# marekrams/tnac4o

Hardware: AMD Instinct MI355X
Metric: PEPS-contraction ms/sweep, chimera L=2048 chi=64 (boundary-MPS sweep _setup_rhoT) (lower is better)
Workload: dtype f64; 1 GPU; chimera L=2048 (Nx=Ny=16, Nc=8), synthetic couplings seed 20260004, beta=3, chi=64; one sweep = 16 rows of MPO absorb + compress_mps; one step = the sweeps of the 4 lattice rotations of one instance; parallelism=1 GPU: 4 lattice rotations of one instance interleaved on 4 HIP streams, mode=sweep

## Files before the change

### tnac4o_amd/csrc/common.h

```cpp
#pragma once
#include <hip/hip_runtime.h>
#include <stdint.h>
#include <stdio.h>
#include <stdlib.h>
#include <string.h>

namespace tn {

void set_error(const char* fmt, ...);
const char* get_error();

inline int hip_fail(hipError_t e, const char* what) {
    set_error("%s: %s", what, hipGetErrorString(e));
    return (int)e > 0 ? (int)e : 1;
}

#define TN_CHECK_ARG(cond, msg)                \
    do {                                       \
        if (!(cond)) {                         \
            tn::set_error("%s: %s", __func__, msg); \
            return -1;                         \
        }                                      \
    } while (0)

#define TN_CHECK_LAUNCH(what)                          \
    do {                                               \
        hipError_t e__ = hipGetLastError();            \
        if (e__ != hipSuccess) return tn::hip_fail(e__, what); \
    } while (0)

inline const char* env_str(const char* name) { return getenv(name); }
inline bool env_flag_on(const char* name) { const char* e = getenv(name); return !(e && e[0] == '0'); }
inline bool env_flag_set(const char* name) { const char* e = getenv(name); return e && e[0] == '1'; }
inline int env_int(const char* name, int dflt) { const char* e = getenv(name); return e ? atoi(e) : dflt; }
inline int64_t env_i64(const char* name, int64_t dflt) { const char* e = getenv(name); return e ? (int64_t)atoll(e) : dflt; }
inline double env_double(const char* name, double dflt) { const char* e = getenv(name); return e ? atof(e) : dflt; }

enum PinSlot {
    PIN_QR = 0,
    PIN_SVD_READ = 2,
    PIN_SVD_UPLOAD = 3,
    PIN_CHAIN_PACK = 4,
    PIN_CHAIN_UPLOAD = 5,
    PIN_CHAIN_READ = 6,
    PIN_SHARED = 7,
    PIN_NSLOTS
};
void* pinned_host(size_t bytes, PinSlot slot);
int read_back(hipStream_t st, void* host, const void* dev, size_t bytes, PinSlot slot, const char* what);
int read_back_staged(hipStream_t st, void** data, const void* dev, size_t bytes, PinSlot slot, const char* what);
int upload(hipStream_t st, void* dev, const void* host, size_t bytes, PinSlot slot, const char* what);

static inline int64_t cdiv(int64_t a, int64_t b) { return (a + b - 1) / b; }
static inline int64_t align_up(int64_t a, int64_t b) { return cdiv(a, b) * b; }

struct WsCarve {
    char* base;
    int64_t off = 0;
    template <typename T = char>
    T* take(int64_t bytes) {
        char* p = base ? base + off : nullptr;
        off += align_up(bytes, 256);
        return (T*)p;
    }
    int64_t total() const { return off; }
};
constexpr int64_t NORMALIZE_SCRATCH_BYTES = 8192;

enum { PROF_GEMM_128x128 = 0, PROF_GEMM_128x32, PROF_GEMM_32x128, PROF_GEMM_64x64, PROF_SPLITK_REDUCE, PROF_ABSORB,
       PROF_GRAM, PROF_EIG, PROF_ROWS_SMALL, PROF_VECS_SMALL,
       PROF_PANEL,
       PROF_LU,
       PROF_QR_AUX,
       PROF_SVD_AUX,
       PROF_MISC,
       PROF_NKERNEL,
       PROF_QR_NOMINAL = PROF_NKERNEL,
       PROF_SVD_NOMINAL,
       PROF_SVD_STREAM,
       PROF_SVDVALS_NOMINAL,
       PROF_SVD_ROUNDS,
       PROF_NFAM };
enum { PH_OTHER = 0, PH_ABSORB, PH_QR, PH_SVD, PH_SVDVALS, PH_BUILD, PH_N };
bool prof_on(int fam);
void prof_begin(hipStream_t st, int fam);
void prof_end(hipStream_t st, int fam, double flops, double bytes);
void prof_note(int fam, double calls, double flops, double bytes);
void prof_note_qr(int64_t m, int64_t n, int64_t batch);
void prof_note_svd(int64_t k, int64_t n, int sweeps);
void prof_note_svdvals(int64_t k, int64_t n);
int prof_phase(int phase);
struct ProfPhase {
    int prev;
    explicit ProfPhase(int ph) : prev(prof_phase(ph)) {}
    ~ProfPhase() { prof_phase(prev); }
};
#define TN_PROF_LAUNCH(st, fam, launch) do { prof_begin(st, fam); launch; prof_end(st, fam, 0.0, 0.0); } while (0)
void prof_set_mask(unsigned mask);
void prof_set_sample(unsigned n);
void prof_reset();
void prof_get(int phase, int fam, uint64_t* calls, double* ms, double* flops, double* bytes);

struct Mat {
    double* p;
    int64_t rs, cs;
};
static inline Mat mat(double* p, int64_t rs, int64_t cs) { return Mat{p, rs, cs}; }
static inline Mat sub(Mat a, int64_t i, int64_t j) { return Mat{a.p + i * a.rs + j * a.cs, a.rs, a.cs}; }
static inline Mat tr(Mat a) { return Mat{a.p, a.cs, a.rs}; }

int gemm(hipStream_t st, int64_t M, int64_t N, int64_t K, double alpha, const double* A, int64_t rsa, int64_t csa,
         const double* B, int64_t rsb, int64_t csb, double beta, double* C, int64_t rsc, int64_t csc,
         int64_t batch = 1, int64_t bsa = 0, int64_t bsb = 0, int64_t bsc = 0, double* ws = nullptr,
         int64_t ws_bytes = 0);
int64_t gemm_ws_bytes(int64_t M, int64_t N, int64_t K, int64_t batch);
struct GemmExtra {
    const int* pairs = nullptr;
    const int* skip = nullptr;
    int pw = 0, mapA = 0, mapB = 0, mapC = 0;
    int force_splitk = 0;
    bool raw_partials = false;
    int* splitk_used = nullptr;
};
int gemm_forced_split(int64_t K, int s, int64_t* kchunk);
int gemm_ex(hipStream_t st, int64_t M, int64_t N, int64_t K, double alpha, const double* A, int64_t rsa, int64_t csa,
            const double* B, int64_t rsb, int64_t csb, double beta, double* C, int64_t rsc, int64_t csc, int64_t batch,
            int64_t bsa, int64_t bsb, int64_t bsc, double* ws, int64_t ws_bytes, const GemmExtra* x);

static inline int gemm(hipStream_t st, int64_t M, int64_t N, int64_t K, double alpha, Mat A, Mat B, double beta, Mat C,
                       double* ws = nullptr, int64_t ws_bytes = 0) {
    return gemm(st, M, N, K, alpha, A.p, A.rs, A.cs, B.p, B.rs, B.cs, beta, C.p, C.rs, C.cs, 1, 0, 0, 0, ws, ws_bytes);
}
int gemm_prof_family(int64_t M, int64_t N, int64_t K, int64_t rsc, int64_t csc);

int rank_update(hipStream_t st, int64_t m, int64_t n, int b, const double* W, int64_t wrs, int64_t wcs, const double* X, int64_t xrs,
                int64_t xcs, double* C, int64_t rsc, int64_t csc, const int* active);
static inline int rank_update(hipStream_t st, int64_t m, int64_t n, int b, Mat W, Mat X, Mat C, const int* active = nullptr) {
    return rank_update(st, m, n, b, W.p, W.rs, W.cs, X.p, X.rs, X.cs, C.p, C.rs, C.cs, active);
}

struct FactorProducts {
    int64_t Z, I, J, K1, N, Mhi, Mlo;
    const double* P; int64_t pz, pi, pk;
    const double* X; int64_t xk, xj, xn;
    const double* W; int64_t wm, wq;
    double* Out; int64_t oz, ohi, olo, on;
};
bool factor_products_fits(int64_t Z, int64_t I, int64_t J, int64_t K1, int64_t N, int64_t M);
inline bool factor_products_on() { return env_flag_on("TN_FACTOR_FUSED"); }
int factor_products(hipStream_t st, const FactorProducts& f);

constexpr int NBMAX = 64;

int gram_partial(hipStream_t st, const double* X, int64_t vs, int64_t es, int64_t L, int nvec, int w, const int* pairs,
                 int ngroups, int nchunk, double* part);
int gram_nchunk(int64_t L);

int eig_small(hipStream_t st, const double* part, int nchunk, int nvec, int ngroups, int mode, int max_sweeps,
              double dead_thresh, double* out, int* dead, int* nrot, double* maxoff, double relevant2 = 0.0, int allow_fast = 1);

int rows_times_small(hipStream_t st, double* X, int64_t rs, int64_t cs, int64_t nrows, int b, const double* S);

struct SvdRoundsJob {
    double* X; int64_t pitch, L; int nvp, w;
    const int* pairs; int ng, nr, nchunk;
    double* part; int64_t part_bytes; double* Js; int* nrot; double* maxoff;
    double relevant2, last_tol; int inner_first, inner_later;
    double* norms;
};
int svd_rounds_fused(hipStream_t st, const SvdRoundsJob& j);
int small_t_times_vecs(hipStream_t st, const double* S, double* X, int64_t vs, int64_t es, int64_t L, int nvec, int w,
                       const int* pairs, int ngroups, const int* nrot);


int qr_factor(hipStream_t st, double* A, int64_t rs, int64_t cs, int64_t m, int64_t n, double* Q, int64_t qrs, int64_t qcs, double* R,
              int64_t rrs, int64_t rcs, int nb, void* ws, int64_t ws_bytes, double rank_tol, int64_t* keff_host,
              double* dropped2_host = nullptr, int frob_exit = 0, int64_t* pivot_perm_host = nullptr, double* nf_out2 = nullptr,
              int* nf_done = nullptr);
int64_t qr_ws_bytes(int64_t m, int64_t n, int nb);


constexpr int CQ_MAXPASS = 4;
constexpr double CQ_THETA = 1e-10;
constexpr double CQ_DONE = 5e-15;
constexpr double CQ_LAST = 1e-8;
int64_t cholqr_ws_bytes(int64_t nrows, int b);
int cholqr_reset(hipStream_t st, void* ws);
int cholqr_begin(hipStream_t st, void* ws, void** state_out);
void cholqr_end_ok(hipStream_t st);
int cholqr_orthonormalize(hipStream_t st, const double* X, int64_t irs, int64_t ics, double* Y, int64_t rs, int64_t cs, int64_t nrows,
                          int b, void* ws, int64_t ws_bytes, uint64_t seed, int* fused_base, void* state = nullptr);
int cholqr_panel(hipStream_t st, const double* X, int64_t irs, int64_t ics, double* Y, int64_t rs, int64_t cs, int64_t nrows, int b, void* ws,
                 int64_t ws_bytes, uint64_t seed, int reconstruct, double* Tp, double* W, int64_t wrs, int64_t wcs, double* Wq, int* fused_base,
                 void* state = nullptr, const int* active = nullptr);
int cholqr_debug_state(hipStream_t st, const void* ws, int* ints9, double* dev_hist);
int cholqr_stats(unsigned long long* out16, int reset, hipStream_t st_or_null, int all_streams);
bool smallqr_fits(int64_t m, int64_t n);
int64_t smallqr_ws_bytes(int64_t m, int64_t n);
int smallqr_factor(hipStream_t st, const double* A, int64_t rs, int64_t cs, int64_t m, int64_t n, double* Q, int64_t qrs, int64_t qcs, double* R,
                   int64_t rrs, int64_t rcs, double* nf_out2, void* ws, int64_t ws_bytes);

constexpr int CQ_FUSED_MAXBLK = 32;
constexpr unsigned CQ_SPIN_LIMIT = 1u << 22;
constexpr int CHOLQR_SLOTS = 64;
int cholqr_stream_slot(hipStream_t st);
void* device_pool_slot(const void* symbol, size_t slot_bytes, int slot);
unsigned panel_spin_limit();
int panel_maxpass();
int fused_maxblk();
bool fused_forms_allowed(hipStream_t st, int nwg);
void fused_forms_disable(hipStream_t st);
void fused_stream_released(hipStream_t st);
struct FusedTallLaunch {
    FusedTallLaunch(hipStream_t st, bool wanted);
    ~FusedTallLaunch();
    FusedTallLaunch(const FusedTallLaunch&) = delete;
// ... 98 lines not shown
```

### tnac4o_amd/csrc/devprim.h

```cpp
#pragma once
#include "common.h"

namespace tn {

static __device__ __forceinline__ double ld_agent(const double* p) { return __hip_atomic_load(p, __ATOMIC_RELAXED, __HIP_MEMORY_SCOPE_AGENT); }
static __device__ __forceinline__ int ldi_agent(const int* p) { return __hip_atomic_load(p, __ATOMIC_RELAXED, __HIP_MEMORY_SCOPE_AGENT); }
static __device__ __forceinline__ void st_agent(double* p, double v) { __hip_atomic_store(p, v, __ATOMIC_RELAXED, __HIP_MEMORY_SCOPE_AGENT); }
static __device__ __forceinline__ void sti_agent(int* p, int v) { __hip_atomic_store(p, v, __ATOMIC_RELAXED, __HIP_MEMORY_SCOPE_AGENT); }
static __device__ __forceinline__ void publish_wait() { __builtin_amdgcn_fence(__ATOMIC_RELEASE, "workgroup"); __builtin_amdgcn_s_waitcnt(0); }

template <int SLEEP>
static __device__ __forceinline__ bool grid_barrier(int* counter, int target, int* s_flag, int tid, unsigned spin_limit, int naps = 0) {
    publish_wait();
    __syncthreads();
    if (tid == 0) {
        atomicAdd(counter, 1);
        int ok = 1;
        unsigned spins = 0;
        while (ldi_agent(counter) < target) {
            __builtin_amdgcn_s_sleep(SLEEP);
            for (int i = 0; i < naps; ++i) __builtin_amdgcn_s_sleep(15);
            if (++spins > spin_limit) { ok = 0; break; }
        }
        *s_flag = ok;
    }
    __syncthreads();
    return *s_flag != 0;
}

static __device__ __forceinline__ double readlane_f64(double v, int lane) {
    int lo = __double2loint(v), hi = __double2hiint(v);
    lo = __builtin_amdgcn_readlane(lo, lane);
    hi = __builtin_amdgcn_readlane(hi, lane);
    return __hiloint2double(hi, lo);
}
static __device__ __forceinline__ double rsqrt2(double x) {
    double r = __builtin_amdgcn_rsq(x);
    r = r * (1.5 - 0.5 * x * r * r);
    r = r * (1.5 - 0.5 * x * r * r);
    return r;
}
static __device__ __forceinline__ double fast_rsqrt(double x) {
    double r = __builtin_amdgcn_rsq(x);
    r = r * (1.5 - 0.5 * x * r * r);
    r = r * (1.5 - 0.5 * x * r * r);
    r = r * (1.5 - 0.5 * x * r * r);
    return r;
}
static __device__ __forceinline__ double fast_rcp(double x) {
    double r = __builtin_amdgcn_rcp(x);
    r = r * (2.0 - x * r);
    r = r * (2.0 - x * r);
    r = r * (2.0 - x * r);
    return r;
}
static __device__ __forceinline__ void fnma(double& acc, double a, double b) {
    asm volatile("v_fma_f64 %0, -%1, %2, %0" : "+v"(acc) : "v"(a), "v"(b));
}
static __device__ __forceinline__ void fnma_s(double& acc, double s_uniform, double v) {
    asm volatile("v_fma_f64 %0, -%1, %2, %0" : "+v"(acc) : "s"(s_uniform), "v"(v));
}
static __device__ __forceinline__ double hash_unit(uint64_t x) {
    x ^= x >> 33; x *= 0xff51afd7ed558ccdULL; x ^= x >> 33; x *= 0xc4ceb9fe1a85ec53ULL; x ^= x >> 33;
    return ((double)(x >> 11) * (1.0 / 9007199254740992.0)) - 0.5;
}
static __device__ __forceinline__ void block_rows(int64_t nrows, int nblk, int blk, int64_t& r0, int& nr) {
    const int64_t base = nrows / nblk, rem = nrows % nblk;
    r0 = blk * base + (blk < rem ? blk : rem);
    nr = (int)(base + (blk < rem ? 1 : 0));
}

static __device__ __forceinline__ double block_sum(double v, double* red, int tid) {
#pragma unroll
    for (int o = 32; o > 0; o >>= 1) v += __shfl_xor(v, o, 64);
    __syncthreads();
    if ((tid & 63) == 0) red[tid >> 6] = v;
    __syncthreads();
    return (red[0] + red[1]) + (red[2] + red[3]);
}
static __device__ __forceinline__ double block_tree_sum(double v, double* red) {
    const int tid = threadIdx.x;
    red[tid] = v;
    __syncthreads();
    for (int k = 128; k > 0; k >>= 1) {
        if (tid < k) red[tid] += red[tid + k];
        __syncthreads();
    }
    const double r = red[0];
    __syncthreads();
    return r;
}
static __device__ __forceinline__ double block_tree_min(double v, double* red) {
    const int tid = threadIdx.x;
    red[tid] = v;
    __syncthreads();
    for (int k = 128; k > 0; k >>= 1) {
        if (tid < k) red[tid] = fmin(red[tid], red[tid + k]);
        __syncthreads();
    }
    const double r = red[0];
    __syncthreads();
    return r;
}

}
```

### tnac4o_amd/csrc/factor_products.hip

```cpp
#include "common.h"

namespace tn {

namespace {

typedef double d4 __attribute__((ext_vector_type(4)));

constexpr int FP_NC = 64;
constexpr int FP_QMAX = 256;
constexpr int FP_IMAX = 16;
constexpr int FP_K1MAX = 64;
constexpr int FP_THREADS = 512, FP_WAVES = FP_THREADS / 64;
constexpr int FP_SLAB = 32 * FP_WAVES;

struct FacP {
    const double* P;
    const double* X;
    const double* W;
    double* Out;
    int Z, I, J, K1, N, M, Mlo, chunks;
    int64_t pz, pi, pk, xk, xj, xn, wm, wq, oz, ohi, olo, on;
};

__device__ __forceinline__ int fp_sidx(int q, int c) { return q * FP_NC + (c ^ ((q & 1) << 4)); }

__device__ __forceinline__ double fp_keep(double v, bool keep) {
    long long m = keep ? -1ll : 0ll;
    asm volatile("" : "+v"(m));
    return __longlong_as_double(__double_as_longlong(v) & m);
}

template <int KS>
__device__ __forceinline__ void fp_stage1(const FacP& g, double* S, const int z, const int n0, const int nb, const int wave, const int lr, const int lk) {
    constexpr int KG = 4 * KS;
    double p[KG];
    {
        const double* Pz = g.P + (int64_t)z * g.pz + (int64_t)min(lr, g.I - 1) * g.pi;
#pragma unroll
        for (int kk = 0; kk < KG; ++kk) {
            const int k = kk * 4 + lk;
            const double v = Pz[(int64_t)min(k, g.K1 - 1) * g.pk];
            p[kk] = fp_keep(v, lr < g.I && k < g.K1);
        }
    }
    const int units = g.J * nb;
    auto load = [&](double (&b)[KG], const int u) {
        const int uc = min(u, units - 1), j = uc / nb, cb = uc - j * nb, n = n0 + cb * 16 + lr;
        const double* Xp = g.X + (int64_t)j * g.xj + (int64_t)min(n, g.N - 1) * g.xn;
#pragma unroll
        for (int kk = 0; kk < KG; ++kk) {
            const int k = kk * 4 + lk;
            const double v = Xp[(int64_t)min(k, g.K1 - 1) * g.xk];
            b[kk] = fp_keep(v, n < g.N && k < g.K1);
        }
    };
    auto multiply = [&](const double (&b)[KG], const int u) {
        if (u >= units) return;
        d4 acc = d4{0.0, 0.0, 0.0, 0.0};
#pragma unroll
        for (int kk = 0; kk < KG; ++kk) acc = __builtin_amdgcn_mfma_f64_16x16x4f64(p[kk], b[kk], acc, 0, 0, 0);
        const int j = u / nb, cb = u - j * nb;
#pragma unroll
        for (int r = 0; r < 4; ++r) {
            const int i = lk + 4 * r;
            if (i < g.I) S[fp_sidx(i * g.J + j, cb * 16 + lr)] = acc[r];
        }
    };
    double b0[KG], b1[KG];
    load(b0, wave);
    for (int u = wave; u < units; u += 2 * FP_WAVES) {
        load(b1, u + FP_WAVES);
        multiply(b0, u);
        load(b0, u + 2 * FP_WAVES);
        multiply(b1, u + FP_WAVES);
    }
}

template <int TN>
__device__ __forceinline__ void fp_stage2(const FacP& g, const double* S, const int z, const int n0, const int Q, const int m0, const int lr, const int lk) {
    const double* Wr[2];
    bool rv[2];
#pragma unroll
    for (int i = 0; i < 2; ++i) {
        const int m = m0 + i * 16 + lr;
        rv[i] = m < g.M;
        Wr[i] = g.W + (int64_t)min(m, g.M - 1) * g.wm;
    }
    auto load = [&](double (&a)[4][2], const int qs) {
#pragma unroll
        for (int kk = 0; kk < 4; ++kk) {
            const int q = qs + kk * 4 + lk;
            const int64_t off = (int64_t)min(q, Q - 1) * g.wq;
#pragma unroll
            for (int i = 0; i < 2; ++i) {
                const double v = Wr[i][off];
                a[kk][i] = fp_keep(v, rv[i] && q < Q);
            }
        }
    };
    d4 acc[2][TN];
#pragma unroll
    for (int i = 0; i < 2; ++i)
#pragma unroll
        for (int j = 0; j < TN; ++j) acc[i][j] = d4{0.0, 0.0, 0.0, 0.0};
    double ac[4][2], an[4][2];
    load(ac, 0);
    for (int qs = 0; qs < Q; qs += 16) {
        load(an, qs + 16);
#pragma unroll
        for (int kk = 0; kk < 4; ++kk) {
            const int q = qs + kk * 4 + lk;
            double b[TN];
#pragma unroll
// ... 87 lines not shown
```

### tnac4o_amd/csrc/gemm_f64.hip

```cpp
#include <stdlib.h>

#include <algorithm>
#include <map>
#include <mutex>
#include <tuple>
#include <vector>

#include "common.h"

namespace tn {

typedef double d4 __attribute__((ext_vector_type(4)));

struct GemmP {
    const double* A;
    const double* B;
    double* C;
    int64_t M, N, K;
    int64_t rsa, csa, rsb, csb, rsc, csc;
    int64_t bsa, bsb, bsc;
    double alpha, beta;
    int splitk;
    int64_t kchunk;
    double* ws;
    int tiles_m, tiles_n;
    const int* pairs;
    const int* skip;
    int pw, mapA, mapB, mapC;
};

constexpr int BK = 16;

template <int BM, int BN, int BKT, bool AKFAST, bool BKFAST, bool MAPPED>
__global__ __launch_bounds__(256, (BM == 128 && BN == 128 && BKT == 16) ? 2 : 1) void gemm_kernel(GemmP g) {
    constexpr int BK = BKT;
    constexpr int PA = BM + 16, PB = BN + 16;
    constexpr int WM = BM / 2, WN = BN / 2, TM = WM / 16, TN = WN / 16;
    constexpr int EA = BM * BK / 256, EB = BN * BK / 256;
    __shared__ double As[2][BK * PA];
    __shared__ double Bs[2][BK * PB];

    const int tid = threadIdx.x, lane = tid & 63, wave = tid >> 6;
    const int wm = wave >> 1, wn = wave & 1;
    int bid = blockIdx.x;
    {
        const int nwg = gridDim.x, q = nwg / 8, r = nwg % 8, xcd = bid % 8, loc = bid / 8;
        bid = (xcd < r ? xcd * (q + 1) : r * (q + 1) + (xcd - r) * q) + loc;
    }
    const int tm0 = (bid / g.tiles_n) * BM, tn0 = (bid % g.tiles_n) * BN;
    const int nsk = g.splitk < 0 ? 1 : g.splitk;
    const int zb = blockIdx.z / nsk, zs = blockIdx.z % nsk;
    if (g.skip && g.skip[zb] == 0) return;
    int blk0 = 0, blk1 = 0;
    if (MAPPED && g.pairs) { blk0 = g.pairs[2 * zb]; blk1 = g.pairs[2 * zb + 1]; }
    auto remap = [&](int64_t v) -> int64_t { return v < g.pw ? (int64_t)blk0 * g.pw + v : (int64_t)blk1 * g.pw + (v - g.pw); };
    const double* A = g.A + zb * g.bsa;
    const double* B = g.B + zb * g.bsb;
    const int64_t k_lo = zs * g.kchunk;
    const int64_t k_hi = (k_lo + g.kchunk < g.K) ? k_lo + g.kchunk : g.K;

    constexpr int DM = AKFAST ? 256 / BK : 0, DKA = AKFAST ? 0 : 256 / BM;
    constexpr int DN = BKFAST ? 256 / BK : 0, DKB = BKFAST ? 0 : 256 / BN;
    const int m0 = AKFAST ? tid / BK : tid % BM, kA0 = AKFAST ? tid % BK : tid / BM;
    const int n0 = BKFAST ? tid / BK : tid % BN, kB0 = BKFAST ? tid % BK : tid / BN;
    const int64_t offA0 = (int64_t)(tm0 + m0) * g.rsa + (int64_t)kA0 * g.csa, stepA = (int64_t)DM * g.rsa + (int64_t)DKA * g.csa;
    const int64_t offB0 = (int64_t)(tn0 + n0) * g.csb + (int64_t)kB0 * g.rsb, stepB = (int64_t)DN * g.csb + (int64_t)DKB * g.rsb;

    double ra[EA], rb[EB];
    auto load_tiles = [&](int64_t k0) {
        if constexpr (!MAPPED) {
            const double* Ak = A + k0 * g.csa + offA0;
            const double* Bk = B + k0 * g.rsb + offB0;
#pragma unroll
            for (int e = 0; e < EA; ++e)
                ra[e] = (tm0 + m0 + e * DM < g.M && k0 + kA0 + e * DKA < k_hi) ? Ak[e * stepA] : 0.0;
#pragma unroll
            for (int e = 0; e < EB; ++e)
                rb[e] = (tn0 + n0 + e * DN < g.N && k0 + kB0 + e * DKB < k_hi) ? Bk[e * stepB] : 0.0;
        } else {
#pragma unroll
            for (int e = 0; e < EA; ++e) {
                const int64_t gm = tm0 + m0 + e * DM, gk = k0 + kA0 + e * DKA;
                ra[e] = (gm < g.M && gk < k_hi) ? A[(g.mapA ? remap(gm) : gm) * g.rsa + gk * g.csa] : 0.0;
            }
#pragma unroll
            for (int e = 0; e < EB; ++e) {
                const int64_t gn = tn0 + n0 + e * DN, gk = k0 + kB0 + e * DKB;
                rb[e] = (gn < g.N && gk < k_hi) ? B[(g.mapB == 1 ? remap(gk) : gk) * g.rsb + (g.mapB == 2 ? remap(gn) : gn) * g.csb] : 0.0;
            }
        }
    };
    auto store_tiles = [&](int stage) {
#pragma unroll
        for (int e = 0; e < EA; ++e) {
            const int m = m0 + e * DM, k = kA0 + e * DKA;
            As[stage][k * PA + (m ^ k)] = ra[e];
        }
#pragma unroll
        for (int e = 0; e < EB; ++e) {
            const int n = n0 + e * DN, k = kB0 + e * DKB;
            Bs[stage][k * PB + (n ^ k)] = rb[e];
        }
    };

    d4 acc[TM][TN];
#pragma unroll
    for (int i = 0; i < TM; ++i)
#pragma unroll
        for (int j = 0; j < TN; ++j) acc[i][j] = d4{0.0, 0.0, 0.0, 0.0};

    const int lr = lane & 15, lk = lane >> 4;
    int cur = 0;
    if (k_lo < k_hi) {
        load_tiles(k_lo);
        store_tiles(0);
    }
    __syncthreads();
    for (int64_t k0 = k_lo; k0 < k_hi; k0 += BK) {
        const bool more = k0 + BK < k_hi;
        if (more) load_tiles(k0 + BK);
        const double* Ac = As[cur];
        const double* Bc = Bs[cur];
#pragma unroll
        for (int kk = 0; kk < BK / 4; ++kk) {
            const int k = kk * 4 + lk;
            double a[TM], b[TN];
#pragma unroll
            for (int i = 0; i < TM; ++i) a[i] = Ac[k * PA + ((wm * WM + i * 16 + lr) ^ k)];
#pragma unroll
            for (int j = 0; j < TN; ++j) b[j] = Bc[k * PB + ((wn * WN + j * 16 + lr) ^ k)];
#pragma unroll
            for (int i = 0; i < TM; ++i)
#pragma unroll
                for (int j = 0; j < TN; ++j)
                    acc[i][j] = __builtin_amdgcn_mfma_f64_16x16x4f64(a[i], b[j], acc[i][j], 0, 0, 0);
        }
        if (more) store_tiles(cur ^ 1);
        __syncthreads();
        cur ^= 1;
    }

    if (g.splitk > 1 || g.splitk < 0) {
        double* W = g.ws + (int64_t)blockIdx.z * g.M * g.N;
#pragma unroll
        for (int i = 0; i < TM; ++i)
#pragma unroll
            for (int j = 0; j < TN; ++j)
#pragma unroll
                for (int r = 0; r < 4; ++r) {
                    const int64_t row = tm0 + wm * WM + i * 16 + lk + 4 * r, col = tn0 + wn * WN + j * 16 + lr;
                    if (row < g.M && col < g.N) W[row * g.N + col] = acc[i][j][r];
                }
    } else {
        double* C = g.C + zb * g.bsc;
        const bool hb = g.beta != 0.0;
        if (hb) {
            double cv[2][TN][4];
            auto fetch = [&](int i, int buf) {
#pragma unroll
                for (int j = 0; j < TN; ++j)
#pragma unroll
                    for (int r = 0; r < 4; ++r) {
                        const int64_t row = tm0 + wm * WM + i * 16 + lk + 4 * r, col = tn0 + wn * WN + j * 16 + lr;
                        cv[buf][j][r] = (row < g.M && col < g.N) ? C[((MAPPED && g.mapC) ? remap(row) : row) * g.rsc + col * g.csc] : 0.0;
                    }
            };
            fetch(0, 0);
#pragma unroll
            for (int i = 0; i < TM; ++i) {
                if (i + 1 < TM) fetch(i + 1, (i + 1) & 1);
#pragma unroll
                for (int j = 0; j < TN; ++j)
#pragma unroll
                    for (int r = 0; r < 4; ++r) {
                        const int64_t row = tm0 + wm * WM + i * 16 + lk + 4 * r, col = tn0 + wn * WN + j * 16 + lr;
                        if (row < g.M && col < g.N) {
                            double v = g.alpha * acc[i][j][r];
                            v += g.beta * cv[i & 1][j][r];
                            C[((MAPPED && g.mapC) ? remap(row) : row) * g.rsc + col * g.csc] = v;
                        }
                    }
            }
        } else {
#pragma unroll
            for (int i = 0; i < TM; ++i)
#pragma unroll
                for (int j = 0; j < TN; ++j)
#pragma unroll
                    for (int r = 0; r < 4; ++r) {
                        const int64_t row = tm0 + wm * WM + i * 16 + lk + 4 * r, col = tn0 + wn * WN + j * 16 + lr;
                        if (row < g.M && col < g.N) C[((MAPPED && g.mapC) ? remap(row) : row) * g.rsc + col * g.csc] = g.alpha * acc[i][j][r];
                    }
        }
    }
}

__global__ __launch_bounds__(256) void splitk_reduce_kernel(GemmP g) {
    const int64_t mn = g.M * g.N;
    const int64_t e = (int64_t)blockIdx.x * 256 + threadIdx.x;
    const int zb = blockIdx.y;
    if (e >= mn) return;
    if (g.skip && g.skip[zb] == 0) return;
    const double* W = g.ws + (int64_t)zb * g.splitk * mn + e;
    double s = 0.0;
    int k = 0;
    for (; k + 8 <= g.splitk; k += 8) {
        double v[8];
#pragma unroll
        for (int u = 0; u < 8; ++u) v[u] = W[(int64_t)(k + u) * mn];
#pragma unroll
        for (int u = 0; u < 8; ++u) s += v[u];
    }
    for (; k < g.splitk; ++k) s += W[(int64_t)k * mn];
    const int64_t row = e / g.N, col = e % g.N;
    double* c = g.C + zb * g.bsc + row * g.rsc + col * g.csc;
    double v = g.alpha * s;
    if (g.beta != 0.0) v += g.beta * *c;
    *c = v;
}

template <int BM, int BN, int BKT>
static void launch_tile(hipStream_t st, const GemmP& g, dim3 grid, bool ak, bool bk) {
    if constexpr (BM == 64 && BN == 64) {
        if (g.pairs) {
            if (ak && bk) hipLaunchKernelGGL((gemm_kernel<BM, BN, BKT, true, true, true>), grid, dim3(256), 0, st, g);
            else if (ak) hipLaunchKernelGGL((gemm_kernel<BM, BN, BKT, true, false, true>), grid, dim3(256), 0, st, g);
            else if (bk) hipLaunchKernelGGL((gemm_kernel<BM, BN, BKT, false, true, true>), grid, dim3(256), 0, st, g);
            else hipLaunchKernelGGL((gemm_kernel<BM, BN, BKT, false, false, true>), grid, dim3(256), 0, st, g);
            return;
        }
    }
    if (ak && bk) hipLaunchKernelGGL((gemm_kernel<BM, BN, BKT, true, true, false>), grid, dim3(256), 0, st, g);
    else if (ak) hipLaunchKernelGGL((gemm_kernel<BM, BN, BKT, true, false, false>), grid, dim3(256), 0, st, g);
    else if (bk) hipLaunchKernelGGL((gemm_kernel<BM, BN, BKT, false, true, false>), grid, dim3(256), 0, st, g);
    else hipLaunchKernelGGL((gemm_kernel<BM, BN, BKT, false, false, false>), grid, dim3(256), 0, st, g);
}

struct GemmPlan { int bm, bn, s; };
static GemmPlan plan_gemm(int64_t M, int64_t N, int64_t K, int64_t batch) {
    static const int64_t small_work = (int64_t)1 << env_int("TN_GEMM_SMALLWORK_LOG2", 30);
    static const int big_tiles = env_int("TN_GEMM_BIGTILES", 1 << 30);
    static const int target_wg = env_int("TN_GEMM_TARGETWG", 256);
    static const int min_chunk = env_int("TN_GEMM_MINCHUNK", 32);
    static const int smax = env_int("TN_GEMM_SMAX", 64);
    static const int bigsplit_wgs = env_int("TN_GEMM_BIGSPLIT_WGS", 192), bigsplit_target = env_int("TN_GEMM_BIGSPLIT_TARGET", 512);
    const bool small = (double)M * (double)N * (double)K * (double)batch < (double)small_work;
    GemmPlan p;
    if (M > 64 && N > 64) {
        const bool big = !small || cdiv(M, 128) * cdiv(N, 128) * batch >= big_tiles;
        p.bm = p.bn = big ? 128 : 64;
    } else if (N <= 32 && M > 64) { p.bm = 128; p.bn = 32; }
    else if (M <= 32 && N > 64) { p.bm = 32; p.bn = 128; }
    else { p.bm = 64; p.bn = 64; }
    const int64_t wgs = cdiv(M, p.bm) * cdiv(N, p.bn) * batch;
    p.s = 1;
    if (small) {
        if (wgs < target_wg * 3 / 4 && K >= 2 * min_chunk) {
            int64_t s = wgs <= 16 ? smax : cdiv(target_wg, wgs);
            if (s > K / min_chunk) s = K / min_chunk;
            if (s > smax) s = smax;
            p.s = s < 2 ? 1 : (int)s;
        }
    } else if (wgs < bigsplit_wgs && K >= 512) {
        int64_t s = cdiv(bigsplit_target, wgs);
        if (s > K / 128) s = K / 128;
        if (s > 64) s = 64;
        p.s = s < 2 ? 1 : (int)s;
    }
    return p;
}

static int tile_family(const GemmPlan& p) {
    return (p.bm == 128 && p.bn == 128) ? PROF_GEMM_128x128 : (p.bm == 128) ? PROF_GEMM_128x32 : (p.bm == 32) ? PROF_GEMM_32x128 : PROF_GEMM_64x64;
}

static bool swaps_roles(int64_t N, int64_t rsc, int64_t csc) {
    static const bool swap_on = env_flag_on("TN_GEMM_SWAP");
    return swap_on && rsc == 1 && csc != 1 && N > 1;
}

int gemm_prof_family(int64_t M, int64_t N, int64_t K, int64_t rsc, int64_t csc) {
    return tile_family(swaps_roles(N, rsc, csc) ? plan_gemm(N, M, K, 1) : plan_gemm(M, N, K, 1));
}

int gemm_forced_split(int64_t K, int s, int64_t* kchunk) {
    *kchunk = s > 1 ? align_up(cdiv(K, s), 2 * BK) : (K > 0 ? align_up(K, 2 * BK) : 2 * BK);
    return s > 1 ? (int)cdiv(K, *kchunk) : s;
}

int64_t gemm_ws_bytes(int64_t M, int64_t N, int64_t K, int64_t batch) {
    const GemmPlan p = plan_gemm(M, N, K, batch);
    return p.s > 1 ? (int64_t)p.s * batch * M * N * 8 : 0;
}

int gemm(hipStream_t st, int64_t M, int64_t N, int64_t K, double alpha, const double* A, int64_t rsa, int64_t csa,
         const double* B, int64_t rsb, int64_t csb, double beta, double* C, int64_t rsc, int64_t csc, int64_t batch,
         int64_t bsa, int64_t bsb, int64_t bsc, double* ws, int64_t ws_bytes) {
    return gemm_ex(st, M, N, K, alpha, A, rsa, csa, B, rsb, csb, beta, C, rsc, csc, batch, bsa, bsb, bsc, ws, ws_bytes, nullptr);
}

namespace {
struct ShapeStat { double ms = 0.0; long calls = 0; };
struct GemmTrace {
    bool on;
    std::mutex mu;
    std::map<std::tuple<int64_t, int64_t, int64_t, int64_t, int, int, int>, ShapeStat> tab;
    GemmTrace() : on(env_flag_set("TN_GEMM_TRACE")) {}
    ~GemmTrace() {
        if (!on || tab.empty()) return;
        std::vector<std::pair<double, std::tuple<int64_t, int64_t, int64_t, int64_t, int, int, int>>> v;
        double tot = 0.0;
        for (auto& kv : tab) { v.push_back({kv.second.ms, kv.first}); tot += kv.second.ms; }
        std::sort(v.begin(), v.end(), [](auto& a, auto& b) { return a.first > b.first; });
        {
            std::map<std::tuple<int, int, int>, ShapeStat> cls;
            for (auto& kv : tab) {
                const int64_t M = std::get<0>(kv.first), N = std::get<1>(kv.first), K = std::get<2>(kv.first), b = std::get<3>(kv.first);
                const int sk = std::get<6>(kv.first);
// ... 7 lines not shown
            for (auto& kv : cls)
                fprintf(stderr, "  %2d %6d %7d : %7ld %9.2f %8.2f\n", std::get<0>(kv.first), std::get<1>(kv.first), std::get<2>(kv.first), kv.second.calls, kv.second.ms,
                        1e3 * kv.second.ms / kv.second.calls);
        }
        fprintf(stderr, "[tn_gemm trace] %zu shapes, %.1f ms in total; M N K batch transA transB splitk : calls, ms, us/call, TFLOP/s\n", v.size(), tot);
        for (size_t i = 0; i < v.size() && i < 40; ++i) {
            auto& k = v[i].second;
            const ShapeStat& st = tab[k];
            const double fl = 2.0 * std::get<0>(k) * std::get<1>(k) * std::get<2>(k) * std::get<3>(k) * st.calls;
            fprintf(stderr, "  %6lld %6lld %6lld %5lld  %d %d %3d : %6ld  %8.2f  %8.2f  %6.2f\n", (long long)std::get<0>(k), (long long)std::get<1>(k),
                    (long long)std::get<2>(k), (long long)std::get<3>(k), std::get<4>(k), std::get<5>(k), std::get<6>(k), st.calls, st.ms,
                    1e3 * st.ms / st.calls, fl / (st.ms * 1e-3) / 1e12);
        }
    }
};
GemmTrace g_trace;
}

static int gemm_ex_impl(hipStream_t st, int64_t M, int64_t N, int64_t K, double alpha, const double* A, int64_t rsa, int64_t csa,
                        const double* B, int64_t rsb, int64_t csb, double beta, double* C, int64_t rsc, int64_t csc, int64_t batch,
                        int64_t bsa, int64_t bsb, int64_t bsc, double* ws, int64_t ws_bytes, const GemmExtra* x);

int gemm_ex(hipStream_t st, int64_t M, int64_t N, int64_t K, double alpha, const double* A, int64_t rsa, int64_t csa,
            const double* B, int64_t rsb, int64_t csb, double beta, double* C, int64_t rsc, int64_t csc, int64_t batch,
            int64_t bsa, int64_t bsb, int64_t bsc, double* ws, int64_t ws_bytes, const GemmExtra* x) {
    if (!g_trace.on) return gemm_ex_impl(st, M, N, K, alpha, A, rsa, csa, B, rsb, csb, beta, C, rsc, csc, batch, bsa, bsb, bsc, ws, ws_bytes, x);
    thread_local hipEvent_t e0 = nullptr, e1 = nullptr;
    if (!e0) { (void)hipEventCreate(&e0); (void)hipEventCreate(&e1); }
    (void)hipEventRecord(e0, st);
    const int rc = gemm_ex_impl(st, M, N, K, alpha, A, rsa, csa, B, rsb, csb, beta, C, rsc, csc, batch, bsa, bsb, bsc, ws, ws_bytes, x);
    (void)hipEventRecord(e1, st);
    (void)hipEventSynchronize(e1);
    float ms = 0.f;
    (void)hipEventElapsedTime(&ms, e0, e1);
    const int sk = (x && x->force_splitk > 0) ? x->force_splitk : plan_gemm(M, N, K, batch).s;
    std::lock_guard<std::mutex> lk(g_trace.mu);
    ShapeStat& ss = g_trace.tab[std::make_tuple(M, N, K, batch, (csa == 1 && rsa != 1) ? 1 : 0, (rsb == 1 && csb != 1) ? 1 : 0, (x && x->pairs) ? -sk : sk)];
    ss.ms += ms;
    ss.calls += 1;
    return rc;
}

static int gemm_ex_impl(hipStream_t st, int64_t M, int64_t N, int64_t K, double alpha, const double* A, int64_t rsa, int64_t csa,
                        const double* B, int64_t rsb, int64_t csb, double beta, double* C, int64_t rsc, int64_t csc, int64_t batch,
                        int64_t bsa, int64_t bsb, int64_t bsc, double* ws, int64_t ws_bytes, const GemmExtra* x) {
    if (M <= 0 || N <= 0 || batch <= 0) return 0;
    TN_CHECK_ARG(K >= 0, "negative K");
    if (swaps_roles(N, rsc, csc) && !(x && (x->pairs || x->raw_partials)))
        return gemm_ex_impl(st, N, M, K, alpha, B, csb, rsb, A, csa, rsa, beta, C, csc, rsc, batch, bsb, bsa, bsc, ws, ws_bytes, x);
    GemmP g;
    g.A = A; g.B = B; g.C = C; g.M = M; g.N = N; g.K = K;
    g.rsa = rsa; g.csa = csa; g.rsb = rsb; g.csb = csb; g.rsc = rsc; g.csc = csc;
    g.bsa = bsa; g.bsb = bsb; g.bsc = bsc; g.alpha = alpha; g.beta = beta; g.ws = ws;
    g.pairs = x ? x->pairs : nullptr; g.skip = x ? x->skip : nullptr;
    g.pw = x ? x->pw : 0; g.mapA = x ? x->mapA : 0; g.mapB = x ? x->mapB : 0; g.mapC = x ? x->mapC : 0;
    const GemmPlan pl = plan_gemm(M, N, K, batch);
    const int bm = pl.bm, bn = pl.bn;
    TN_CHECK_ARG(g.pairs == nullptr || (bm == 64 && bn == 64), "block-pair indirection is built for the 64 x 64 tile only");
    g.tiles_m = (int)cdiv(M, bm); g.tiles_n = (int)cdiv(N, bn);
    int s = (x && x->force_splitk > 0) ? x->force_splitk : pl.s;
    if (s > 1) {
        const int64_t fit = ws ? ws_bytes / (batch * M * N * 8) : 0;
        if (fit < s) s = fit < 2 ? 1 : (int)fit;
    }
    const bool raw = x && x->raw_partials;
    TN_CHECK_ARG(!raw || ws != nullptr, "raw partials need a workspace");
    g.splitk = s = gemm_forced_split(K, s, &g.kchunk);
    if (raw && s == 1) g.splitk = -1;
    if (x && x->splitk_used) *x->splitk_used = s;
    if (batch * s > 65535) {
        TN_CHECK_ARG(x == nullptr && s <= 65535, "batch*splitk exceeds grid.z");
        const int64_t cb = 65535 / s;
        for (int64_t b0 = 0; b0 < batch; b0 += cb) {
            const int64_t nbt = batch - b0 < cb ? batch - b0 : cb;
            const int rc = gemm_ex_impl(st, M, N, K, alpha, A + b0 * bsa, rsa, csa, B + b0 * bsb, rsb, csb, beta, C + b0 * bsc, rsc, csc,
                                        nbt, bsa, bsb, bsc, ws, ws_bytes, nullptr);
            if (rc) return rc;
        }
        return 0;
    }
    const bool ak = (csa == 1 && rsa != 1), bk = (rsb == 1 && csb != 1);
    dim3 grid(g.tiles_m * g.tiles_n, 1, (unsigned)(batch * s));
    const int fam = tile_family(pl);
    prof_begin(st, fam);
    if (bm == 128 && bn == 128) launch_tile<128, 128, 16>(st, g, grid, ak, bk);
    else if (bm == 128 && bn == 32) launch_tile<128, 32, 16>(st, g, grid, ak, bk);
    else if (bm == 32 && bn == 128) launch_tile<32, 128, 16>(st, g, grid, ak, bk);
    else launch_tile<64, 64, 16>(st, g, grid, ak, bk);
    TN_CHECK_LAUNCH("gemm_kernel");
    prof_end(st, fam, 2.0 * M * N * K * batch, 8.0 * batch * ((double)M * K + (double)K * N + (double)M * N));
    if (s > 1 && !raw) {
        dim3 rg((unsigned)cdiv(M * N, 256), (unsigned)batch);
        prof_begin(st, PROF_SPLITK_REDUCE);
        hipLaunchKernelGGL(splitk_reduce_kernel, rg, dim3(256), 0, st, g);
        TN_CHECK_LAUNCH("splitk_reduce_kernel");
        prof_end(st, PROF_SPLITK_REDUCE, (double)s * M * N * batch, 8.0 * batch * ((double)s + 1.0) * M * N);
    }
    return 0;
}

}
```

Before: 362.2 ms/sweep.

## Add register-prefetch pipelined 64x64 GEMM path with clamped branchless loads

Adds a PIPE variant of the 64x64 GEMM kernel, selected by default when the K range is at least 128 and no block-pair mapping is used. Global loads for the next two K-tiles are issued into registers before the MFMA work on the current tile. Bounds checks become clamped addresses plus a bitmask that zeroes out-of-range values, so every load is unconditional. Scheduling barriers keep loads ahead of the compute, and the launch bound asks for two workgroups per CU. This aims to hide global-memory latency in the mid-size GEMMs, at the cost of more registers and more code in the kernel.

```diff
diff --git a/tnac4o_amd/csrc/common.h b/tnac4o_amd/csrc/common.h
--- a/tnac4o_amd/csrc/common.h
+++ b/tnac4o_amd/csrc/common.h
@@ -80,6 +80,7 @@
        PROF_SVD_STREAM,
        PROF_SVDVALS_NOMINAL,
        PROF_SVD_ROUNDS,
+       PROF_GEMM_PIPE,
        PROF_NFAM };
 enum { PH_OTHER = 0, PH_ABSORB, PH_QR, PH_SVD, PH_SVDVALS, PH_BUILD, PH_N };
 bool prof_on(int fam);
@@ -132,6 +133,8 @@
     return gemm(st, M, N, K, alpha, A.p, A.rs, A.cs, B.p, B.rs, B.cs, beta, C.p, C.rs, C.cs, 1, 0, 0, 0, ws, ws_bytes);
 }
 int gemm_prof_family(int64_t M, int64_t N, int64_t K, int64_t rsc, int64_t csc);
+
+inline bool gemm_pipe_selected(int fam, int64_t krange) { return fam == PROF_GEMM_64x64 && krange >= 128; }
 
 int rank_update(hipStream_t st, int64_t m, int64_t n, int b, const double* W, int64_t wrs, int64_t wcs, const double* X, int64_t xrs,
                 int64_t xcs, double* C, int64_t rsc, int64_t csc, const int* active);
diff --git a/tnac4o_amd/csrc/devprim.h b/tnac4o_amd/csrc/devprim.h
--- a/tnac4o_amd/csrc/devprim.h
+++ b/tnac4o_amd/csrc/devprim.h
@@ -33,6 +33,11 @@
     lo = __builtin_amdgcn_readlane(lo, lane);
     hi = __builtin_amdgcn_readlane(hi, lane);
     return __hiloint2double(hi, lo);
+}
+static __device__ __forceinline__ double fp_keep(double v, bool keep) {
+    long long m = keep ? -1ll : 0ll;
+    asm volatile("" : "+v"(m));
+    return __longlong_as_double(__double_as_longlong(v) & m);
 }
 static __device__ __forceinline__ double rsqrt2(double x) {
     double r = __builtin_amdgcn_rsq(x);
diff --git a/tnac4o_amd/csrc/factor_products.hip b/tnac4o_amd/csrc/factor_products.hip
--- a/tnac4o_amd/csrc/factor_products.hip
+++ b/tnac4o_amd/csrc/factor_products.hip
@@ -1,4 +1,4 @@
-#include "common.h"
+#include "devprim.h"
 
 namespace tn {
 
@@ -23,12 +23,6 @@
 };
 
 __device__ __forceinline__ int fp_sidx(int q, int c) { return q * FP_NC + (c ^ ((q & 1) << 4)); }
-
-__device__ __forceinline__ double fp_keep(double v, bool keep) {
-    long long m = keep ? -1ll : 0ll;
-    asm volatile("" : "+v"(m));
-    return __longlong_as_double(__double_as_longlong(v) & m);
-}
 
 template <int KS>
 __device__ __forceinline__ void fp_stage1(const FacP& g, double* S, const int z, const int n0, const int nb, const int wave, const int lr, const int lk) {
diff --git a/tnac4o_amd/csrc/gemm_f64.hip b/tnac4o_amd/csrc/gemm_f64.hip
--- a/tnac4o_amd/csrc/gemm_f64.hip
+++ b/tnac4o_amd/csrc/gemm_f64.hip
@@ -6,7 +6,8 @@
 #include <tuple>
 #include <vector>
 
-#include "common.h"
+#include "devprim.h"
+#include "gemm_index.h"
 
 namespace tn {
 
@@ -31,8 +32,9 @@
 
 constexpr int BK = 16;
 
-template <int BM, int BN, int BKT, bool AKFAST, bool BKFAST, bool MAPPED>
-__global__ __launch_bounds__(256, (BM == 128 && BN == 128 && BKT == 16) ? 2 : 1) void gemm_kernel(GemmP g) {
+template <int BM, int BN, int BKT, bool AKFAST, bool BKFAST, bool MAPPED, bool PIPE>
+__global__ __launch_bounds__(256, ((BM == 128 && BN == 128 && BKT == 16) || PIPE) ? 2 : 1) void gemm_kernel(GemmP g) {
+    static_assert(!(PIPE && MAPPED), "the pipelined loop has no block-pair indirection");
     constexpr int BK = BKT;
     constexpr int PA = BM + 16, PB = BN + 16;
     constexpr int WM = BM / 2, WN = BN / 2, TM = WM / 16, TN = WN / 16;
@@ -110,17 +112,9 @@
         for (int j = 0; j < TN; ++j) acc[i][j] = d4{0.0, 0.0, 0.0, 0.0};
 
     const int lr = lane & 15, lk = lane >> 4;
-    int cur = 0;
-    if (k_lo < k_hi) {
-        load_tiles(k_lo);
-        store_tiles(0);
-    }
-    __syncthreads();
-    for (int64_t k0 = k_lo; k0 < k_hi; k0 += BK) {
-        const bool more = k0 + BK < k_hi;
-        if (more) load_tiles(k0 + BK);
-        const double* Ac = As[cur];
-        const double* Bc = Bs[cur];
+    auto multiply = [&](int stage) {
+        const double* Ac = As[stage];
+        const double* Bc = Bs[stage];
 #pragma unroll
         for (int kk = 0; kk < BK / 4; ++kk) {
             const int k = kk * 4 + lk;
@@ -135,9 +129,70 @@
                 for (int j = 0; j < TN; ++j)
                     acc[i][j] = __builtin_amdgcn_mfma_f64_16x16x4f64(a[i], b[j], acc[i][j], 0, 0, 0);
         }
-        if (more) store_tiles(cur ^ 1);
+    };
+    if constexpr (!PIPE) {
+        int cur = 0;
+        if (k_lo < k_hi) {
+            load_tiles(k_lo);
+            store_tiles(0);
+        }
         __syncthreads();
-        cur ^= 1;
+        for (int64_t k0 = k_lo; k0 < k_hi; k0 += BK) {
+            const bool more = k0 + BK < k_hi;
+            if (more) load_tiles(k0 + BK);
+            multiply(cur);
+            if (more) store_tiles(cur ^ 1);
+            __syncthreads();
+            cur ^= 1;
+        }
+    } else if (k_lo < k_hi) {
+        GemmClampedWalk<BM, BK, AKFAST> wa;
+        GemmClampedWalk<BN, BK, BKFAST> wb;
+        typedef typename decltype(wa)::T TA;
+        typedef typename decltype(wb)::T TB;
+        static_assert(TA::E == EA && TB::E == EB && TA::D == DM && TA::DK == DKA && TB::D == DN && TB::DK == DKB, "gemm_index.h describes this tile map");
+        wa.init(tm0, tid, g.M, k_hi, g.rsa, g.csa);
+        wb.init(tn0, tid, g.N, k_hi, g.csb, g.rsb);
+        double pa[2][EA], pb[2][EB];
+        auto issue = [&](int set, int64_t k0) {
+#pragma unroll
+            for (int e = 0; e < EA; ++e) pa[set][e] = A[wa.at(e, k0).off];
+#pragma unroll
+            for (int e = 0; e < EB; ++e) pb[set][e] = B[wb.at(e, k0).off];
+        };
+        auto stash = [&](int set, int stage, int64_t k0) {
+#pragma unroll
+            for (int e = 0; e < EA; ++e) {
+                const int m = m0 + e * DM, k = kA0 + e * DKA;
+                As[stage][k * PA + (m ^ k)] = fp_keep(pa[set][e], wa.at(e, k0).keep);
+            }
+#pragma unroll
+            for (int e = 0; e < EB; ++e) {
+                const int n = n0 + e * DN, k = kB0 + e * DKB;
+                Bs[stage][k * PB + (n ^ k)] = fp_keep(pb[set][e], wb.at(e, k0).keep);
+            }
+        };
+        issue(0, k_lo);
+        issue(1, k_lo + BK);
+        __builtin_amdgcn_sched_barrier(0);
+        stash(0, 0, k_lo);
+        __syncthreads();
+        int64_t k0 = k_lo;
+        for (; k0 + BK < k_hi; k0 += 2 * BK) {
+            issue(0, k0 + 2 * BK);
+            __builtin_amdgcn_sched_barrier(0);
+            multiply(0);
+            __builtin_amdgcn_sched_barrier(0);
+            stash(1, 1, k0 + BK);
+            __syncthreads();
+            issue(1, k0 + 3 * BK);
+            __builtin_amdgcn_sched_barrier(0);
+            multiply(1);
+            __builtin_amdgcn_sched_barrier(0);
+            stash(0, 0, k0 + 2 * BK);
+            __syncthreads();
+        }
+        if (k0 < k_hi) multiply(0);
     }
 
     if (g.splitk > 1 || g.splitk < 0) {
@@ -219,21 +274,23 @@
     *c = v;
 }
 
+template <int BM, int BN, int BKT, bool MAPPED, bool PIPE>
+static void launch_layout(hipStream_t st, const GemmP& g, dim3 grid, bool ak, bool bk) {
+    if (ak && bk) hipLaunchKernelGGL((gemm_kernel<BM, BN, BKT, true, true, MAPPED, PIPE>), grid, dim3(256), 0, st, g);
+    else if (ak) hipLaunchKernelGGL((gemm_kernel<BM, BN, BKT, true, false, MAPPED, PIPE>), grid, dim3(256), 0, st, g);
+    else if (bk) hipLaunchKernelGGL((gemm_kernel<BM, BN, BKT, false, true, MAPPED, PIPE>), grid, dim3(256), 0, st, g);
+    else hipLaunchKernelGGL((gemm_kernel<BM, BN, BKT, false, false, MAPPED, PIPE>), grid, dim3(256), 0, st, g);
+}
+
 template <int BM, int BN, int BKT>
-static void launch_tile(hipStream_t st, const GemmP& g, dim3 grid, bool ak, bool bk) {
+static void launch_tile(hipStream_t st, const GemmP& g, dim3 grid, bool ak, bool bk, bool pipe) {
     if constexpr (BM == 64 && BN == 64) {
-        if (g.pairs) {
-            if (ak && bk) hipLaunchKernelGGL((gemm_kernel<BM, BN, BKT, true, true, true>), grid, dim3(256), 0, st, g);
-            else if (ak) hipLaunchKernelGGL((gemm_kernel<BM, BN, BKT, true, false, true>), grid, dim3(256), 0, st, g);
-            else if (bk) hipLaunchKernelGGL((gemm_kernel<BM, BN, BKT, false, true, true>), grid, dim3(256), 0, st, g);
-            else hipLaunchKernelGGL((gemm_kernel<BM, BN, BKT, false, false, true>), grid, dim3(256), 0, st, g);
-            return;
-        }
-    }
-    if (ak && bk) hipLaunchKernelGGL((gemm_kernel<BM, BN, BKT, true, true, false>), grid, dim3(256), 0, st, g);
-    else if (ak) hipLaunchKernelGGL((gemm_kernel<BM, BN, BKT, true, false, false>), grid, dim3(256), 0, st, g);
-    else if (bk) hipLaunchKernelGGL((gemm_kernel<BM, BN, BKT, false, true, false>), grid, dim3(256), 0, st, g);
-    else hipLaunchKernelGGL((gemm_kernel<BM, BN, BKT, false, false, false>), grid, dim3(256), 0, st, g);
+        if (g.pairs) return launch_layout<BM, BN, BKT, true, false>(st, g, grid, ak, bk);
+    }
+    if constexpr (BM == 64 && BN == 64) {
+        if (pipe) return launch_layout<BM, BN, BKT, false, true>(st, g, grid, ak, bk);
+    }
+    launch_layout<BM, BN, BKT, false, false>(st, g, grid, ak, bk);
 }
 
 struct GemmPlan { int bm, bn, s; };
@@ -407,12 +464,15 @@
     const bool ak = (csa == 1 && rsa != 1), bk = (rsb == 1 && csb != 1);
     dim3 grid(g.tiles_m * g.tiles_n, 1, (unsigned)(batch * s));
     const int fam = tile_family(pl);
+    const int pipe_mode = env_int("TN_GEMM_PIPE", 1);
+    const bool pipe = fam == PROF_GEMM_64x64 && !g.pairs && (pipe_mode >= 2 || (pipe_mode == 1 && gemm_pipe_selected(fam, s > 1 ? g.kchunk : K)));
     prof_begin(st, fam);
-    if (bm == 128 && bn == 128) launch_tile<128, 128, 16>(st, g, grid, ak, bk);
-    else if (bm == 128 && bn == 32) launch_tile<128, 32, 16>(st, g, grid, ak, bk);
-    else if (bm == 32 && bn == 128) launch_tile<32, 128, 16>(st, g, grid, ak, bk);
-    else launch_tile<64, 64, 16>(st, g, grid, ak, bk);
+    if (bm == 128 && bn == 128) launch_tile<128, 128, 16>(st, g, grid, ak, bk, pipe);
+    else if (bm == 128 && bn == 32) launch_tile<128, 32, 16>(st, g, grid, ak, bk, pipe);
+    else if (bm == 32 && bn == 128) launch_tile<32, 128, 16>(st, g, grid, ak, bk, pipe);
+    else launch_tile<64, 64, 16>(st, g, grid, ak, bk, pipe);
     TN_CHECK_LAUNCH("gemm_kernel");
+    if (pipe) prof_note(PROF_GEMM_PIPE, 1, 0.0, 0.0);
     prof_end(st, fam, 2.0 * M * N * K * batch, 8.0 * batch * ((double)M * K + (double)K * N + (double)M * N));
     if (s > 1 && !raw) {
         dim3 rg((unsigned)cdiv(M * N, 256), (unsigned)batch);
diff --git a/tnac4o_amd/csrc/gemm_index.h b/tnac4o_amd/csrc/gemm_index.h
--- /dev/null
+++ b/tnac4o_amd/csrc/gemm_index.h
@@ -0,0 +1,77 @@
+#pragma once
+#include <stdint.h>
+
+#if defined(__HIPCC__) || defined(__CUDACC__)
+#define TN_HD __host__ __device__ __forceinline__
+#else
+#define TN_HD inline
+#endif
+
+namespace tn {
+
+template <int BT, int BKT, bool KFAST>
+struct GemmTileMap {
+    static constexpr int E = BT * BKT / 256;
+    static constexpr int D = KFAST ? 256 / BKT : 0, DK = KFAST ? 0 : 256 / BT;
+    static TN_HD int i0(int tid) { return KFAST ? tid / BKT : tid % BT; }
+    static TN_HD int kk0(int tid) { return KFAST ? tid % BKT : tid / BT; }
+};
+
+struct GemmLoad {
+    int64_t off;
+    bool keep;
+};
+
+template <int BT, int BKT, bool KFAST>
+TN_HD GemmLoad gemm_guarded_index(int t0, int tid, int e, int64_t k0, int64_t dim, int64_t k_hi, int64_t s_dim, int64_t s_k) {
+    typedef GemmTileMap<BT, BKT, KFAST> T;
+    const int64_t gi = t0 + T::i0(tid) + e * T::D, gk = k0 + T::kk0(tid) + e * T::DK;
+    return GemmLoad{gi * s_dim + gk * s_k, gi < dim && gk < k_hi};
+}
+
+TN_HD int64_t gemm_clamped_part(int64_t g, int64_t n, int64_t stride) { return (g < n ? g : n - 1) * stride; }
+template <int BT, int BKT, bool KFAST>
+TN_HD GemmLoad gemm_clamped_index(int t0, int tid, int e, int64_t k0, int64_t dim, int64_t k_hi, int64_t s_dim, int64_t s_k) {
+    typedef GemmTileMap<BT, BKT, KFAST> T;
+    const int64_t gi = t0 + T::i0(tid) + e * T::D, gk = k0 + T::kk0(tid) + e * T::DK;
+    return GemmLoad{gemm_clamped_part(gi, dim, s_dim) + gemm_clamped_part(gk, k_hi, s_k), gi < dim && gk < k_hi};
+}
+
+template <int BT, int BKT, bool KFAST>
+struct GemmClampedWalk {
+    typedef GemmTileMap<BT, BKT, KFAST> T;
+    static constexpr int NI = KFAST ? T::E : 1;
+    int64_t ipart[NI];
+    bool iok[NI];
+    int kk0;
+    int64_t kofs, kstep, klast, s_k, k_hi;
+    TN_HD void init(int t0, int tid, int64_t dim, int64_t k_hi_, int64_t s_dim, int64_t s_k_) {
+#pragma unroll
+        for (int e = 0; e < NI; ++e) {
+            const int64_t gi = t0 + T::i0(tid) + e * T::D;
+            ipart[e] = gemm_clamped_part(gi, dim, s_dim);
+            iok[e] = gi < dim;
+        }
+        kk0 = T::kk0(tid);
+        s_k = s_k_;
+        k_hi = k_hi_;
+        kofs = kk0 * s_k;
+        kstep = T::DK * s_k;
+        klast = (k_hi - 1) * s_k;
+    }
+    TN_HD GemmLoad at(int e, int64_t k0) const {
+        const bool kin = k0 + kk0 + e * T::DK < k_hi;
+        return GemmLoad{ipart[KFAST ? e : 0] + pick(kin, k0 * s_k + kofs + e * kstep, klast), iok[KFAST ? e : 0] && kin};
+    }
+    static TN_HD int64_t pick(bool c, int64_t a, int64_t b) {
+#if defined(__HIP_DEVICE_COMPILE__)
+        long long m = c ? -1ll : 0ll;
+        asm volatile("" : "+v"(m));
+        return b ^ ((a ^ b) & m);
+#else
+        return c ? a : b;
+#endif
+    }
+};
+
+}
```

Result: no change. 365.0 ms/sweep (+0.8%).
